# DaanVrancken/HubbardTN

Hardware: AMD Instinct MI355X
Metric: DMRG sweep time (s) + GS energy/site, 1-band Hubbard L=64 chi=1024 (lower is better)
Workload: dtype c128; 1 GPU; one-band Hubbard chain L=64 U/t=4, half filling, fZ2xSU(2)xU(1), two-site DMRG sweep (2L-3=125 bond updates) at chi=1024 (TensorKit dim units); model=one_band, L=64, chi=1024, krylovdim=30, parallelism=sector-parallel apply x1, backend=hip

## Files before the change

### hubbardtn_amd/csrc/htn_svd.hip

```cpp
#include <algorithm>
#include <map>
#include <memory>
#include <mutex>
#include <vector>

#include "htn_common.h"

#define JAC_THREADS 1024
#define JAC_MAXEL 8

template <int GS>
__device__ __forceinline__ double group_sum(double v) {
    v = row_sum16(v);
    if (GS == 16) return v;
    const double a = lane_bcast<0>(v) + lane_bcast<16>(v);
    const double b = lane_bcast<32>(v) + lane_bcast<48>(v);
    if (GS == 32) return (threadIdx.x & 32) ? b : a;
    return a + b;
}

template <int GS>
__device__ __forceinline__ double jacobi_pair(double2* ga, double2* gb, double2* __restrict__ va,
                                              double2* __restrict__ vb, int m, int n, int sub, double tol,
                                              bool accumulate, double zero2) {
// ... 342 lines not shown
    bool local;
    double2* qn;
    int* scol;
    double* cn2;
    int* meta;
    unsigned* qflag;
    unsigned* hflag;
    unsigned* fail;
};
__device__ __forceinline__ bool qr_wait_ge(unsigned* flag, unsigned want, unsigned* fail) {
    const long long t0 = wall_clock64();
    for (unsigned spins = 1;; ++spins) {
        if (__hip_atomic_load(flag, __ATOMIC_RELAXED, __HIP_MEMORY_SCOPE_AGENT) >= want) return true;
        __builtin_amdgcn_s_sleep(1);
        if ((spins & 255u) == 0u) {
            if (__hip_atomic_load(fail, __ATOMIC_RELAXED, __HIP_MEMORY_SCOPE_AGENT) != 0u) return false;
            if (wall_clock64() - t0 > 300000000ll) {
                __hip_atomic_store(fail, 1u, __ATOMIC_RELAXED, __HIP_MEMORY_SCOPE_AGENT);
                return false;
            }
        }
    }
}
template <bool SH>
__device__ __forceinline__ double2 qr_ld(const double2* base, __amdgpu_buffer_rsrc_t rs, int idx) {
    if (!SH) return base[idx];
    const qr_u4 u = __builtin_amdgcn_raw_buffer_load_b128(rs, idx * 16, 0, 16);
    double2 v;
    __builtin_memcpy(&v, &u, 16);
    return v;
}
template <bool SH>
__device__ __forceinline__ void qr_st(double2* base, __amdgpu_buffer_rsrc_t rs, int idx, double2 v, bool local) {
    if (!SH) {
        base[idx] = v;
        return;
    }
    qr_u4 u;
    __builtin_memcpy(&u, &v, 16);
    if (local) __builtin_amdgcn_raw_buffer_store_b128(u, rs, idx * 16, 0, 0);
    else __builtin_amdgcn_raw_buffer_store_b128(u, rs, idx * 16, 0, 16);
}

template <bool SH>
__device__ __forceinline__ void qr_trailing_chunk(double2* __restrict__ g0, __amdgpu_buffer_rsrc_t rg, double2* __restrict__ Xg,
                                                  __amdgpu_buffer_rsrc_t rx, const double2* Qn, int ldq, const int* s_col, int m0,
                                                  int m0p, int n0, int mp, int j0, int nb_eff, int k_first, int ch, bool last_panel,
                                                  double* norm_out, bool norm_shared, int lane, bool local) {
    const int l15 = lane & 15, l4 = lane >> 4;
    const int nks = m0p >> 2;
    const int k = k_first + 16 * ch + l15;
    const bool valid = k < n0;
    const int pk = valid ? s_col[k] : 0;
    const int abase = pk * m0;
    d4 cr = {0.0, 0.0, 0.0, 0.0}, ci = {0.0, 0.0, 0.0, 0.0};
    const double2* qrow = Qn + l15 * ldq + l4;
    double2 ring[4];
#pragma unroll
    for (int u = 0; u < 4; ++u) {
        const int i = 4 * u + l4;
        ring[u] = (valid && u < nks && i < m0) ? qr_ld<SH>(g0, rg, abase + i) : make_double2(0.0, 0.0);
    }
    for (int ks0 = 0; ks0 < nks; ks0 += 4) {
#pragma unroll
        for (int u = 0; u < 4; ++u) {
            const int ks = ks0 + u;
            if (ks < nks) {
                const double2 b = ring[u];
                const int inx = 4 * (ks + 4) + l4;
                ring[u] = (valid && ks + 4 < nks && inx < m0) ? qr_ld<SH>(g0, rg, abase + inx) : make_double2(0.0, 0.0);
                const double2 qv = qrow[4 * ks];
                cr = __builtin_amdgcn_mfma_f64_16x16x4f64(qv.x, b.x, cr, 0, 0, 0);
                ci = __builtin_amdgcn_mfma_f64_16x16x4f64(qv.x, b.y, ci, 0, 0, 0);
                cr = __builtin_amdgcn_mfma_f64_16x16x4f64(qv.y, b.y, cr, 0, 0, 0);
                ci = __builtin_amdgcn_mfma_f64_16x16x4f64(-qv.y, b.x, ci, 0, 0, 0);
            }
        }
    }
#pragma unroll
    for (int reg = 0; reg < 4; ++reg) {
        const int t = l4 + 4 * reg;
        if (valid && t < nb_eff) qr_st<SH>(Xg, rx, (j0 + t) * mp + pk, make_double2(cr[reg], -ci[reg]), local);
    }
    if (last_panel) return;
    double nrm = 0.0;
    for (int i0 = 0; i0 < m0p; i0 += 16) {
        double2 old[4];
#pragma unroll
        for (int reg = 0; reg < 4; ++reg) {
            const int i = i0 + l4 + 4 * reg;
            old[reg] = (valid && i < m0) ? qr_ld<SH>(g0, rg, abase + i) : make_double2(0.0, 0.0);
        }
        d4 dr = {0.0, 0.0, 0.0, 0.0}, di = {0.0, 0.0, 0.0, 0.0};
#pragma unroll
        for (int kk = 0; kk < 4; ++kk) {
            const double2 qa = Qn[(l4 + 4 * kk) * ldq + i0 + l15];
            dr = __builtin_amdgcn_mfma_f64_16x16x4f64(qa.x, cr[kk], dr, 0, 0, 0);
            di = __builtin_amdgcn_mfma_f64_16x16x4f64(qa.x, ci[kk], di, 0, 0, 0);
            dr = __builtin_amdgcn_mfma_f64_16x16x4f64(-qa.y, ci[kk], dr, 0, 0, 0);
            di = __builtin_amdgcn_mfma_f64_16x16x4f64(qa.y, cr[kk], di, 0, 0, 0);
        }
#pragma unroll
        for (int reg = 0; reg < 4; ++reg) {
            const int i = i0 + l4 + 4 * reg;
            if (valid && i < m0) {
                const double2 x = make_double2(old[reg].x - dr[reg], old[reg].y - di[reg]);
                qr_st<SH>(g0, rg, abase + i, x, local);
                nrm += x.x * x.x + x.y * x.y;
            }
        }
    }
    nrm += __shfl_xor(nrm, 16, 64);
    nrm += __shfl_xor(nrm, 32, 64);
    if (valid && l4 == 0) {
        if (norm_shared) __hip_atomic_store(norm_out + k, nrm, __ATOMIC_RELAXED, __HIP_MEMORY_SCOPE_AGENT);
        else norm_out[k] = nrm;
    }
}

template <bool SH>
__device__ __forceinline__ void qr_trailing_coop(double2* __restrict__ g0, __amdgpu_buffer_rsrc_t rg, double2* __restrict__ Xg,
                                                 __amdgpu_buffer_rsrc_t rx, const double2* Qn, int ldq, const int* s_col, int m0,
                                                 int m0p, int n0, int mp, int j0, int nb_eff, int k_first, int nchunks, int role,
                                                 int NW, bool last_panel, double* norm_out, bool norm_shared, double* part,
                                                 int tid, bool local) {
    __shared__ double s_np[JAC_THREADS / 64][16];
    const int lane = tid & 63, wave = tid >> 6, l15 = lane & 15, l4 = lane >> 4;
    const int cnt = nchunks > role ? (nchunks - role + NW - 1) / NW : 0;
    if (part == nullptr) {
        for (int q = wave; q < cnt; q += JAC_THREADS / 64)
            qr_trailing_chunk<SH>(g0, rg, Xg, rx, Qn, ldq, s_col, m0, m0p, n0, mp, j0, nb_eff, k_first, role + NW * q, last_panel, norm_out,
                                  norm_shared, lane, local);
        return;
    }
    constexpr int S = 4, CPR = (JAC_THREADS / 64) / S;
    const int nks = m0p >> 2;
    for (int r0 = 0; r0 < cnt; r0 += CPR) {
        const int ci_ = r0 + wave / S, pp = wave % S;
        const bool act = ci_ < cnt;
        const int ch = role + NW * ci_;
        const int k = k_first + 16 * ch + l15;
        const bool valid = act && k < n0;
        const int pk = valid ? s_col[k] : 0;
        const int abase = pk * m0;
        d4 cr = {0.0, 0.0, 0.0, 0.0}, ci = {0.0, 0.0, 0.0, 0.0};
        if (act) {
            const double2* qrow = Qn + l15 * ldq + l4;
            double2 ring[4];
#pragma unroll
            for (int u = 0; u < 4; ++u) {
                const int ks = 4 * pp + u, i = 4 * ks + l4;
                ring[u] = (valid && ks < nks && i < m0) ? qr_ld<SH>(g0, rg, abase + i) : make_double2(0.0, 0.0);
            }
            for (int ks0 = 4 * pp; ks0 < nks; ks0 += 4 * S) {
#pragma unroll
                for (int u = 0; u < 4; ++u) {
                    const int ks = ks0 + u;
                    if (ks < nks) {
                        const double2 b = ring[u];
                        const int ksn = ks + 4 * S, inx = 4 * ksn + l4;
                        ring[u] = (valid && ksn < nks && inx < m0) ? qr_ld<SH>(g0, rg, abase + inx) : make_double2(0.0, 0.0);
                        const double2 qv = qrow[4 * ks];
                        cr = __builtin_amdgcn_mfma_f64_16x16x4f64(qv.x, b.x, cr, 0, 0, 0);
                        ci = __builtin_amdgcn_mfma_f64_16x16x4f64(qv.x, b.y, ci, 0, 0, 0);
                        cr = __builtin_amdgcn_mfma_f64_16x16x4f64(qv.y, b.y, cr, 0, 0, 0);
                        ci = __builtin_amdgcn_mfma_f64_16x16x4f64(-qv.y, b.x, ci, 0, 0, 0);
                    }
                }
            }
        }
        {
            double* mine = part + (size_t)wave * 512 + lane;
#pragma unroll
            for (int reg = 0; reg < 4; ++reg) {
                mine[64 * reg] = cr[reg];
                mine[64 * (4 + reg)] = ci[reg];
            }
        }
        __syncthreads();
        {
            const double* base = part + (size_t)(wave - pp) * 512 + lane;
#pragma unroll
            for (int reg = 0; reg < 4; ++reg) {
                double a = 0.0, b = 0.0;
#pragma unroll
                for (int q = 0; q < S; ++q) {
                    a += base[q * 512 + 64 * reg];
                    b += base[q * 512 + 64 * (4 + reg)];
                }
                cr[reg] = a;
                ci[reg] = b;
            }
        }
        if (pp == 0) {
#pragma unroll
            for (int reg = 0; reg < 4; ++reg) {
                const int t = l4 + 4 * reg;
                if (valid && t < nb_eff) qr_st<SH>(Xg, rx, (j0 + t) * mp + pk, make_double2(cr[reg], -ci[reg]), local);
            }
        }
        if (!last_panel) {
            double nrm = 0.0;
            if (act) {
                for (int i0 = 16 * pp; i0 < m0p; i0 += 16 * S) {
                    double2 old[4];
#pragma unroll
                    for (int reg = 0; reg < 4; ++reg) {
                        const int i = i0 + l4 + 4 * reg;
                        old[reg] = (valid && i < m0) ? qr_ld<SH>(g0, rg, abase + i) : make_double2(0.0, 0.0);
                    }
                    d4 dr = {0.0, 0.0, 0.0, 0.0}, di = {0.0, 0.0, 0.0, 0.0};
#pragma unroll
                    for (int kk = 0; kk < 4; ++kk) {
                        const double2 qa = Qn[(l4 + 4 * kk) * ldq + i0 + l15];
                        dr = __builtin_amdgcn_mfma_f64_16x16x4f64(qa.x, cr[kk], dr, 0, 0, 0);
                        di = __builtin_amdgcn_mfma_f64_16x16x4f64(qa.x, ci[kk], di, 0, 0, 0);
                        dr = __builtin_amdgcn_mfma_f64_16x16x4f64(-qa.y, ci[kk], dr, 0, 0, 0);
                        di = __builtin_amdgcn_mfma_f64_16x16x4f64(qa.y, cr[kk], di, 0, 0, 0);
                    }
#pragma unroll
                    for (int reg = 0; reg < 4; ++reg) {
                        const int i = i0 + l4 + 4 * reg;
                        if (valid && i < m0) {
                            const double2 x = make_double2(old[reg].x - dr[reg], old[reg].y - di[reg]);
                            qr_st<SH>(g0, rg, abase + i, x, local);
                            nrm += x.x * x.x + x.y * x.y;
                        }
                    }
                }
            }
            nrm += __shfl_xor(nrm, 16, 64);
            nrm += __shfl_xor(nrm, 32, 64);
            if (l4 == 0) s_np[wave][l15] = nrm;
            __syncthreads();
            if (valid && pp == 0 && l4 == 0) {
                double t = 0.0;
#pragma unroll
                for (int q = 0; q < S; ++q) t += s_np[wave + q][l15];
                if (norm_shared) __hip_atomic_store(norm_out + k, t, __ATOMIC_RELAXED, __HIP_MEMORY_SCOPE_AGENT);
                else norm_out[k] = t;
            }
        }
        __syncthreads();
    }
}

__device__ __forceinline__ void qr_helper(double2* __restrict__ g0, int m0, int n0, int r, double2* __restrict__ Xg, int mp, int* s_col,
                                          double2* Qn, int tid, const QrShare sh, double* part) {
    __shared__ int s_meta[8];
    const int lane = tid & 63, wave = tid >> 6;
    const int m0p = (m0 + 15) & ~15, ldq = m0p + 1;
    const __amdgpu_buffer_rsrc_t rg = __builtin_amdgcn_make_buffer_rsrc((void*)g0, 0, m0 * n0 * 16, 0x00020000);
    const __amdgpu_buffer_rsrc_t rx = __builtin_amdgcn_make_buffer_rsrc((void*)Xg, 0, mp * r * 16, 0x00020000);
    const __amdgpu_buffer_rsrc_t rq = __builtin_amdgcn_make_buffer_rsrc((void*)sh.qn, 0, 16 * ldq * 16, 0x00020000);
    for (unsigned epoch = 1;; ++epoch) {
        if (tid == 0) {
            const bool ok = qr_wait_ge(sh.qflag, epoch, sh.fail);
            s_meta[5] = ok ? 0 : 1;
            for (int q = 0; q < 5; ++q) s_meta[q] = ok ? __hip_atomic_load(sh.meta + q, __ATOMIC_RELAXED, __HIP_MEMORY_SCOPE_AGENT) : 0;
        }
        __syncthreads();
        const int j0 = s_meta[0], nb_eff = s_meta[1], k_first = s_meta[2];
        const bool last_panel = s_meta[3] != 0, finished = s_meta[4] != 0 || s_meta[5] != 0;
        if (finished) break;
        for (int idx = tid; idx < 16 * ldq; idx += JAC_THREADS) Qn[idx] = qr_ld<true>(sh.qn, rq, idx);
        for (int k = k_first + tid; k < n0; k += JAC_THREADS) s_col[k] = __hip_atomic_load(sh.scol + k, __ATOMIC_RELAXED, __HIP_MEMORY_SCOPE_AGENT);
        __syncthreads();
        const int nchunks = (n0 - k_first + 15) >> 4;
        qr_trailing_coop<true>(g0, rg, Xg, rx, Qn, ldq, s_col, m0, m0p, n0, mp, j0, nb_eff, k_first, nchunks, sh.role, sh.NW, last_panel, sh.cn2,
                               true, part, tid, sh.local);
        asm volatile("s_waitcnt vmcnt(0)" ::: "memory");
        __syncthreads();
        if (tid == 0) __hip_atomic_store(sh.hflag + sh.role, epoch, __ATOMIC_RELAXED, __HIP_MEMORY_SCOPE_AGENT);
    }
}

#ifdef HTN_QR_PROF
__device__ long long g_qr_prof[8];
extern "C" int htn_qr_prof_dump(long long* out) {
    HIP_TRY(hipDeviceSynchronize());
    HIP_TRY(hipMemcpyFromSymbol(out, HIP_SYMBOL(g_qr_prof), sizeof(long long) * 8));
    return 0;
}
#define QR_T(var) const long long var = wall_clock64()
#define QR_ACC(slot, a, b) qprof[slot] += (b) - (a)
#else
#define QR_T(var)
#define QR_ACC(slot, a, b)
#endif
template <int EL, bool SH>
__device__ __forceinline__ int qrcp_blocked(double2* __restrict__ g0, int m0, int n0, int r,
                                            double2* __restrict__ Xg, int mp, int* s_col, double* s_cn2,
                                            double* s_piv, double2* Qn, int tid, double cut2, const QrShare sh, double* part) {
    __shared__ double s_pn[16];
    __shared__ int s_share_ok;
    const __amdgpu_buffer_rsrc_t rg = __builtin_amdgcn_make_buffer_rsrc((void*)g0, 0, m0 * n0 * 16, 0x00020000);
    const __amdgpu_buffer_rsrc_t rx = __builtin_amdgcn_make_buffer_rsrc((void*)Xg, 0, mp * r * 16, 0x00020000);
    unsigned pub_epoch = 0;
    if (tid == 0) s_share_ok = 1;
    __shared__ double2 s_r[16][17];
    __shared__ int s_pc[16];
    __shared__ int s_pos[16];
    __shared__ int s_nb;
    const int lane = tid & 63, wave = tid >> 6, l15 = lane & 15, l4 = lane >> 4;
    const int m0p = (m0 + 15) & ~15, ldq = m0p + 1;
    for (int idx = tid; idx < mp * r; idx += JAC_THREADS) qr_st<SH>(Xg, rx, idx, make_double2(0.0, 0.0), sh.local);
    for (int k = wave; k < n0; k += JAC_THREADS / 64) {
        double c = 0.0;
        for (int i = lane; i < m0; i += 64) {
            const double2 x = g0[(int64_t)k * m0 + i];
            c += x.x * x.x + x.y * x.y;
        }
        c = wave_sum(c);
        if (lane == 0) {
            s_cn2[k] = c;
            s_col[k] = k;
        }
    }
    __syncthreads();
    if (wave == 0) {
        double f = 0.0;
        for (int k = lane; k < n0; k += 64) f += s_cn2[k];
        f = wave_sum(f);
        if (lane == 0) s_piv[1] = 1e-30 * f;
    }
    __syncthreads();
    const double zero2 = s_piv[1];
    bool stop = false;
    int j0 = 0, rank = 0;
#ifdef HTN_QR_PROF
    long long qprof[8] = {0, 0, 0, 0, 0, 0, 0, 0};
    const long long qt0 = wall_clock64();
#endif
    while (j0 < r && !stop) {
        QR_T(q0);
        const int nbmax = r - j0 < 16 ? r - j0 : 16;
        if (wave == 0) {
            int nb = 0;
            double mass = 0.0;
            for (int k = j0 + lane; k < n0; k += 64) mass += s_cn2[k];
            mass = wave_sum(mass);
            for (int t = 0; t < (mass <= cut2 ? 0 : nbmax); ++t) {
                const int j = j0 + t;
                unsigned long long key = 0ull;
                for (int k = j + lane; k < n0; k += 64) {
                    const unsigned long long kk =
                        ((unsigned long long)__double_as_longlong(s_cn2[k]) & ~0x3FFull) | (unsigned long long)(1023 - k);
                    key = kk > key ? kk : key;
                }
                key = wave_max_u64(key);
                const int bi = 1023 - (int)(key & 0x3FFull);
                const double best = s_cn2[bi];
                if (best <= zero2) break;
                if (lane == 0) {
                    const int tc = s_col[j];
                    s_col[j] = s_col[bi];
                    s_col[bi] = tc;
                    s_cn2[bi] = s_cn2[j];
                    s_cn2[j] = best;
                }
                ++nb;
            }
            if (lane == 0) s_nb = nb;
        }
        __syncthreads();
        QR_T(q1);
        QR_ACC(0, q0, q1);
        int nb = s_nb;
        if (nb == 0) break;
        if (nb < nbmax) stop = true;
        const bool owner = wave < nb;
        const int pc = owner ? s_col[j0 + wave] : 0;
        double2 a[EL];
        double cn = owner ? s_cn2[j0 + wave] : -1.0;
        const double ns = cn;
#pragma unroll
        for (int e = 0; e < EL; ++e) {
            const int i = lane + 64 * e;
            a[e] = (owner && i < m0) ? qr_ld<SH>(g0, rg, pc * m0 + i) : make_double2(0.0, 0.0);
        }
        if (!owner)
            for (int i = lane; i < m0p; i += 64) Qn[wave * ldq + i] = make_double2(0.0, 0.0);
        if (tid < 256) s_r[tid >> 4][tid & 15] = make_double2(0.0, 0.0);
        if (lane == 0) s_pc[wave] = pc;
        bool pending = owner;
        int nb_eff = nb;
        QR_T(q2);
        QR_ACC(1, q1, q2);
        for (int t = 0; t < nb; ++t) {
            if (lane == 0) s_pn[wave] = pending ? cn : -1.0;
            lds_barrier();
            unsigned long long key = 0ull;
            {
                const double v = s_pn[l15];
                if (v >= 0.0) key = ((unsigned long long)__double_as_longlong(v) & ~0xFull) | (unsigned long long)(15 - l15);
            }
            key = row_max16_u64(key);
            const int bu = 15 - (int)(key & 0xFull);
            const double best = key ? s_pn[bu] : -1.0;
            if (best <= zero2) {
                nb_eff = t;
                stop = true;
                break;
            }
            if (wave == bu) {
                if (cn < 1e-4 * ns) {
                    for (int s2 = 0; s2 < t; ++s2) {
                        double dr = 0.0, di = 0.0;
                        const double2* qs = Qn + s2 * ldq + lane;
#pragma unroll
                        for (int e = 0; e < EL; ++e) {
                            if (lane + 64 * e < m0p) {
                                const double2 q = qs[64 * e];
                                dr += q.x * a[e].x + q.y * a[e].y;
                                di += q.x * a[e].y - q.y * a[e].x;
                            }
                        }
                        dr = wave_sum(dr);
                        di = wave_sum(di);
#pragma unroll
                        for (int e = 0; e < EL; ++e) {
                            if (lane + 64 * e < m0p) {
                                const double2 q = qs[64 * e];
                                a[e].x -= dr * q.x - di * q.y;
                                a[e].y -= dr * q.y + di * q.x;
                            }
                        }
                        if (lane == 0) {
                            const double2 old = s_r[s2][wave];
                            s_r[s2][wave] = make_double2(old.x + dr, old.y - di);
                        }
                    }
                    double c = 0.0;
#pragma unroll
                    for (int e = 0; e < EL; ++e) c += a[e].x * a[e].x + a[e].y * a[e].y;
                    cn = wave_sum(c);
                }
                const double ipn = fast_rsq(cn);
                const double pn = cn * ipn;
#pragma unroll
                for (int e = 0; e < EL; ++e) {
                    const int i = lane + 64 * e;
                    if (i < m0p) Qn[t * ldq + i] = make_double2(a[e].x * ipn, a[e].y * ipn);
                }
                if (lane == 0) {
                    s_r[t][wave] = make_double2(pn, 0.0);
                    s_pos[t] = pc;
                }
                pending = false;
            }
            lds_barrier();
            if (pending) {
                double dr = 0.0, di = 0.0;
                const double2* qt = Qn + t * ldq + lane;
#pragma unroll
                for (int e = 0; e < EL; ++e) {
                    if (lane + 64 * e < m0p) {
                        const double2 q = qt[64 * e];
                        dr += q.x * a[e].x + q.y * a[e].y;
                        di += q.x * a[e].y - q.y * a[e].x;
                    }
                }
                dr = wave_sum(dr);
                di = wave_sum(di);
                double c = 0.0;
#pragma unroll
                for (int e = 0; e < EL; ++e) {
                    if (lane + 64 * e < m0p) {
                        const double2 q = qt[64 * e];
                        a[e].x -= dr * q.x - di * q.y;
                        a[e].y -= dr * q.y + di * q.x;
                        c += a[e].x * a[e].x + a[e].y * a[e].y;
                    }
                }
                cn = wave_sum(c);
                if (lane == 0) s_r[t][wave] = make_double2(dr, -di);
            }
        }
        __syncthreads();
        QR_T(q3);
        QR_ACC(2, q2, q3);
        if (nb_eff < nb) {
            for (int tt = nb_eff + wave; tt < nb; tt += JAC_THREADS / 64)
                for (int i = lane; i < m0p; i += 64) Qn[tt * ldq + i] = make_double2(0.0, 0.0);
        }
        if (tid < nb_eff) s_col[j0 + tid] = s_pos[tid];
        if (tid < 256 && (tid >> 4) < nb_eff && (tid & 15) < nb)
            qr_st<SH>(Xg, rx, (j0 + (tid >> 4)) * mp + s_pc[tid & 15], s_r[tid >> 4][tid & 15], sh.local);
        __syncthreads();
        QR_T(q4);
        QR_ACC(3, q3, q4);
        const int k_first = j0 + nb;
        const int nchunks = (n0 - k_first + 15) >> 4;
        const bool last_panel = stop || k_first >= r;
        const int NW = SH ? sh.NW : 1;
        if (SH && nchunks > 0) {
            const __amdgpu_buffer_rsrc_t rq = __builtin_amdgcn_make_buffer_rsrc((void*)sh.qn, 0, 16 * ldq * 16, 0x00020000);
            for (int idx = tid; idx < 16 * ldq; idx += JAC_THREADS) qr_st<true>(sh.qn, rq, idx, Qn[idx], sh.local);
            for (int k = k_first + tid; k < n0; k += JAC_THREADS) __hip_atomic_store(sh.scol + k, s_col[k], __ATOMIC_RELAXED, __HIP_MEMORY_SCOPE_AGENT);
            if (tid == 0) {
                __hip_atomic_store(sh.meta + 0, j0, __ATOMIC_RELAXED, __HIP_MEMORY_SCOPE_AGENT);
                __hip_atomic_store(sh.meta + 1, nb_eff, __ATOMIC_RELAXED, __HIP_MEMORY_SCOPE_AGENT);
                __hip_atomic_store(sh.meta + 2, k_first, __ATOMIC_RELAXED, __HIP_MEMORY_SCOPE_AGENT);
                __hip_atomic_store(sh.meta + 3, last_panel ? 1 : 0, __ATOMIC_RELAXED, __HIP_MEMORY_SCOPE_AGENT);
                __hip_atomic_store(sh.meta + 4, 0, __ATOMIC_RELAXED, __HIP_MEMORY_SCOPE_AGENT);
            }
            asm volatile("s_waitcnt vmcnt(0)" ::: "memory");
            __syncthreads();
            ++pub_epoch;
            if (tid == 0) __hip_atomic_store(sh.qflag, pub_epoch, __ATOMIC_RELAXED, __HIP_MEMORY_SCOPE_AGENT);
        }
        qr_trailing_coop<SH>(g0, rg, Xg, rx, Qn, ldq, s_col, m0, m0p, n0, mp, j0, nb_eff, k_first, nchunks, 0, NW, last_panel, s_cn2, false, part,
                             tid, sh.local);
        if (SH && nchunks > 0) {
            asm volatile("s_waitcnt vmcnt(0)" ::: "memory");
            __syncthreads();
            if (tid == 0) {
                bool ok = true;
                for (int h = 1; h < NW && ok; ++h) ok = qr_wait_ge(sh.hflag + h, pub_epoch, sh.fail);
                if (!ok) s_share_ok = 0;
            }
            __syncthreads();
            if (!s_share_ok) {
                stop = true;
            } else if (!last_panel) {
                for (int k = k_first + tid; k < n0; k += JAC_THREADS)
                    if (((k - k_first) >> 4) % NW != 0) s_cn2[k] = __hip_atomic_load(sh.cn2 + k, __ATOMIC_RELAXED, __HIP_MEMORY_SCOPE_AGENT);
            }
        }
        __syncthreads();
        QR_T(q5);
        QR_ACC(4, q4, q5);
#ifdef HTN_QR_PROF
        qprof[6] += 1;
#endif
        j0 += nb;
        rank += nb_eff;
    }
    __syncthreads();
#ifdef HTN_QR_PROF
    if (tid == 0 && blockIdx.x == 0) {
        qprof[5] = wall_clock64() - qt0;
        for (int q = 0; q < 8; ++q) g_qr_prof[q] = qprof[q];
    }
#endif
    if (SH) {
        if (tid == 0) {
            __hip_atomic_store(sh.meta + 4, 1, __ATOMIC_RELAXED, __HIP_MEMORY_SCOPE_AGENT);
            asm volatile("s_waitcnt vmcnt(0)" ::: "memory");
            __hip_atomic_store(sh.qflag, pub_epoch + 1, __ATOMIC_RELAXED, __HIP_MEMORY_SCOPE_AGENT);
        }
        __syncthreads();
        if (!s_share_ok) rank = -1;
    }
    for (int i = tid; i < n0; i += JAC_THREADS) s_col[i] = i;
    __syncthreads();
    return rank;
}

#define QR_SYNC_WORDS 16
#define QR_BOX_BYTES 137728
__global__ __launch_bounds__(JAC_THREADS) void k_qr_large(double2* __restrict__ G, double2* __restrict__ Vj,
                                                          const htn_svd_block* __restrict__ desc,
                                                          const int* __restrict__ large_ids, int* __restrict__ perm,
                                                          double* __restrict__ zero2_out, double cut2,
                                                          int* __restrict__ rank_host, int NW, char* __restrict__ qr_box,
                                                          unsigned* __restrict__ qr_sync, int nl, int nx, int part_off) {
    extern __shared__ double2 g_lds[];
    __shared__ double s_piv[2];
    __shared__ int s_col[64 * JAC_MAXEL];
    __shared__ double s_cn2[64 * JAC_MAXEL];
    __shared__ int s_qlocal;
    const int px = (int)(blockIdx.x % (unsigned)nx), ps = (int)(blockIdx.x / (unsigned)nx);
    const int li = (ps / NW) * nx + px, role = ps % NW;
    if (li >= nl) return;
    const htn_svd_block D = desc[large_ids[li]];
    const int m = D.m, n = D.n, m0 = D.pad, tid = threadIdx.x;
    const int gsx = m <= 16 * JAC_MAXEL ? 16 : (m <= 32 * JAC_MAXEL ? 32 : 64);
    const int mp = gsx * ((m + gsx - 1) / gsx);
    double2* __restrict__ X = Vj + D.v_off;
    QrShare sh;
    sh.NW = NW, sh.role = role;
    char* box = qr_box + (size_t)li * QR_BOX_BYTES;
    sh.qn = (double2*)box;
    sh.scol = (int*)(box + 16 * 513 * 16);
    sh.cn2 = (double*)(box + 16 * 513 * 16 + 512 * 4);
    sh.meta = (int*)(box + 16 * 513 * 16 + 512 * 4 + 512 * 8);
    sh.qflag = qr_sync + li * QR_SYNC_WORDS;
    sh.hflag = qr_sync + li * QR_SYNC_WORDS + 1;
    sh.fail = qr_sync + nl * QR_SYNC_WORDS;
    sh.local = false;
    if (NW > 1) {
        if (tid == 0) {
            unsigned xcc;
            asm volatile("s_getreg_b32 %0, hwreg(HW_REG_XCC_ID)" : "=s"(xcc));
            xcc = (xcc & 0xfu) + 1u;
            unsigned* xw = qr_sync + li * QR_SYNC_WORDS + 8;
            __hip_atomic_store(xw + role, xcc, __ATOMIC_RELAXED, __HIP_MEMORY_SCOPE_AGENT);
            int local = 1;
            for (int q = 0; q < NW && local >= 0; ++q) {
                if (!qr_wait_ge(xw + q, 1u, sh.fail)) local = -1;
                else if (__hip_atomic_load(xw + q, __ATOMIC_RELAXED, __HIP_MEMORY_SCOPE_AGENT) != xcc) local = 0;
            }
            s_qlocal = local;
        }
        __syncthreads();
        sh.local = s_qlocal > 0;
    }
    double* part = (part_off > 0 && ((m0 + 15) & ~15) <= 256) ? (double*)(g_lds + part_off) : nullptr;
    if (role > 0) {
        qr_helper(G + D.g_off, m0, m, n, X, mp, s_col, (double2*)g_lds, tid, sh, part);
        return;
    }
    int rank;
    if (NW > 1) {
        if (m0 <= 256) rank = qrcp_blocked<4, true>(G + D.g_off, m0, m, n, X, mp, s_col, s_cn2, s_piv, (double2*)g_lds, tid, cut2, sh, part);
        else rank = qrcp_blocked<8, true>(G + D.g_off, m0, m, n, X, mp, s_col, s_cn2, s_piv, (double2*)g_lds, tid, cut2, sh, part);
    } else {
        if (m0 <= 256) rank = qrcp_blocked<4, false>(G + D.g_off, m0, m, n, X, mp, s_col, s_cn2, s_piv, (double2*)g_lds, tid, cut2, sh, part);
        else rank = qrcp_blocked<8, false>(G + D.g_off, m0, m, n, X, mp, s_col, s_cn2, s_piv, (double2*)g_lds, tid, cut2, sh, part);
    }
    if (tid == 0) {
        rank_host[li] = rank;
        zero2_out[li] = s_piv[1];
        __threadfence_system();
    }
    for (int i = tid; i < m; i += JAC_THREADS) perm[li * 64 * JAC_MAXEL + i] = s_col[i];
}

__global__ __launch_bounds__(JAC_THREADS) void k_jacobi_svd(double2* __restrict__ G, double2* __restrict__ Vj,
                                                            double* __restrict__ S,
                                                            const htn_svd_block* __restrict__ desc,
                                                            int max_sweeps, double tol, int* __restrict__ info,
                                                            int lds_elems, const int* __restrict__ large_slot,
                                                            double cut2) {
    extern __shared__ double2 g_lds[];
    __shared__ double s_ratio;
    __shared__ double s_piv[2];
    __shared__ int s_col[64 * JAC_MAXEL];
    __shared__ double s_cn2[64 * JAC_MAXEL];
    if (large_slot && large_slot[blockIdx.x] >= 0) return;
    const htn_svd_block D = desc[blockIdx.x];
    const int m = D.m, n = D.n;
    double2* __restrict__ gglob = G + D.g_off;
    double2* __restrict__ v = Vj + D.v_off;
// ... 1507 lines not shown
```

Measured before the change: 423.5 ms.

## Parallelize QRCP pivot-block selection with block-wide top-17 rank merge

```diff
diff --git a/hubbardtn_amd/csrc/htn_svd.hip b/hubbardtn_amd/csrc/htn_svd.hip
--- a/hubbardtn_amd/csrc/htn_svd.hip
+++ b/hubbardtn_amd/csrc/htn_svd.hip
@@ -668,6 +668,9 @@
     __shared__ int s_pc[16];
     __shared__ int s_pos[16];
     __shared__ int s_nb;
+    unsigned long long (*s_wcand)[17] = reinterpret_cast<unsigned long long (*)[17]>(&s_r[0][0]);
+    unsigned long long* s_wsel = &s_wcand[16][0];
+    static_assert(sizeof(s_r) >= sizeof(unsigned long long) * 17 * 17, "window keys alias s_r");
     const int lane = tid & 63, wave = tid >> 6, l15 = lane & 15, l4 = lane >> 4;
     const int m0p = (m0 + 15) & ~15, ldq = m0p + 1;
     for (int idx = tid; idx < mp * r; idx += JAC_THREADS) qr_st<SH>(Xg, rx, idx, make_double2(0.0, 0.0), sh.local);
@@ -701,12 +704,82 @@
     while (j0 < r && !stop) {
         QR_T(q0);
         const int nbmax = r - j0 < 16 ? r - j0 : 16;
+        double mass = 0.0;
+        {
+            const int cnt = n0 - j0, S = (cnt + 15) >> 4;
+            const int k = j0 + wave * S + lane;
+            const bool in = lane < S && k < n0;
+            const unsigned long long key =
+                in ? (((unsigned long long)__double_as_longlong(s_cn2[k]) & ~0x3FFull) | (unsigned long long)(1023 - k)) : 0ull;
+            int rk = 0;
+            for (int s = 0; s < S; ++s) {
+                const unsigned long long o = ((unsigned long long)(unsigned)__builtin_amdgcn_readlane((int)(key >> 32), s) << 32) |
+                                             (unsigned)__builtin_amdgcn_readlane((int)(unsigned)key, s);
+                rk += o > key ? 1 : 0;
+            }
+            if (wave == 0) {
+                for (int kk = j0 + lane; kk < n0; kk += 64) mass += s_cn2[kk];
+                mass = wave_sum(mass);
+            }
+            if (lane < 17) s_wcand[wave][lane] = 0ull;
+            if (in && rk < 17) s_wcand[wave][rk] = key;
+            if (tid < 17) s_wsel[tid] = 0ull;
+            lds_barrier();
+            if (tid < 16 * 17) {
+                const unsigned long long x = s_wcand[tid / 17][tid % 17];
+                int c[16];
+#pragma unroll
+                for (int w = 0; w < 16; ++w) c[w] = 0;
+#pragma unroll
+                for (int st = 16; st > 0; st >>= 1) {
+                    unsigned long long v[16];
+#pragma unroll
+                    for (int w = 0; w < 16; ++w) v[w] = s_wcand[w][c[w] + st - 1 < 17 ? c[w] + st - 1 : 16];
+#pragma unroll
+                    for (int w = 0; w < 16; ++w) c[w] += (c[w] + st - 1 < 17 && v[w] > x) ? st : 0;
+                }
+                int g = 0;
+#pragma unroll
+                for (int w = 0; w < 16; ++w) g += c[w];
+                if (x != 0ull && g < 17) s_wsel[g] = x;
+            }
+            lds_barrier();
+        }
         if (wave == 0) {
             int nb = 0;
-            double mass = 0.0;
-            for (int k = j0 + lane; k < n0; k += 64) mass += s_cn2[k];
-            mass = wave_sum(mass);
-            for (int t = 0; t < (mass <= cut2 ? 0 : nbmax); ++t) {
+            const int nbw = mass <= cut2 ? 0 : nbmax;
+            const int K = nbw + 1 < n0 - j0 ? nbw + 1 : n0 - j0;
+            const unsigned long long sk = lane < 17 ? s_wsel[lane] : 0ull;
+            const unsigned long long sn = lane < 16 ? s_wsel[lane + 1] : 0ull;
+            const bool tie = __ballot(lane + 1 < K && (sk >> 10) == (sn >> 10)) != 0ull;
+            if (!tie) {
+                const int p = 1023 - (int)(sk & 0x3FFull);
+                nb = __popcll(__ballot(lane < nbw && sk != 0ull && s_cn2[sk != 0ull ? p : j0] > zero2));
+                const int u = lane & 15;
+                const unsigned long long su = s_wsel[u];
+                int cur = 1023 - (int)(su & 0x3FFull), bi = 0;
+                for (int t = 0; t < nb; ++t) {
+                    const int b = __builtin_amdgcn_readlane(cur, t);
+                    if (u == t) bi = b;
+                    if (u > t && cur == j0 + t) cur = b;
+                }
+                const bool act = lane < 32 && u < nb;
+                const int x = lane < 16 ? j0 + u : bi;
+                int y = x;
+                for (int t = nb - 1; t >= 0; --t) {
+                    const int b = __builtin_amdgcn_readlane(bi, t);
+                    y = y == j0 + t ? b : (y == b ? j0 + t : y);
+                }
+                const int c = act ? s_col[y] : 0;
+                const double v = act ? s_cn2[y] : 0.0;
+                if (act) {
+                    s_col[x] = c;
+                    s_cn2[x] = v;
+                }
+            } else for (int t = 0; t < nbw; ++t) {
+#ifdef HTN_QR_PROF
+                if (t == 0 && lane == 0) qprof[7] += 1;
+#endif
                 const int j = j0 + t;
                 unsigned long long key = 0ull;
                 for (int k = j + lane; k < n0; k += 64) {
```

After: 426.0 ms, median of 2. No clear change (+0.6%).
